# liuyuan-pal/NeRO

Measured on AMD Instinct MI355X. Metric: training rays/sec (Stage-I shape, 128 samples/ray), higher is better.
Workload: dtype f32 (dense layers: fp32 operands carried as exact / block-scaled 16-bit plane pairs or triples on the bf16/fp16 matrix pipe with fp32 accumulation, fp32-grade error; modes {'fwd': 'f16x3', 'tan': 'f16x3', 'bwd': 'f16x3', 'dw': 'f16x3'}); 1 GPU; GlossySynthetic 'bell' Stage-I shape, 4096 rays x (64+64+32) samples per GPU, training-schedule step 25000; rays_per_gpu=4096, parallelism=dp1, optimizer=adam(fused), streams=3, f16_paired_mask=3, fg_table=reference asset (tests/golden/fg_lut_ref.npz)

## Files before the change

nero_amd/csrc/mlp_f16_util.h:

```cpp
#pragma once

#ifdef F16_PHASE_TIMING
__device__ unsigned long long g_phase[16];
#define PH_DECL long long ph_t = clock64(), ph_acc[8] = {0, 0, 0, 0, 0, 0, 0, 0}
#define PH(k) do { __builtin_amdgcn_sched_barrier(0); const long long t_ = clock64(); ph_acc[k] += t_ - ph_t; ph_t = t_; __builtin_amdgcn_sched_barrier(0); } while (0)
#define PH_PARAM , long long& ph_t, long long (&ph_acc)[8]
#define PH_ARG , ph_t, ph_acc
#define PH_END do { if (threadIdx.x == 0) for (int k_ = 0; k_ < 8; ++k_) atomicAdd(&g_phase[k_], (unsigned long long)ph_acc[k_]); } while (0)
#else
#define PH_PARAM
#define PH_ARG
#define PH_DECL
#define PH(k)
#define PH_END
#endif

typedef _Float16 f16x8 __attribute__((ext_vector_type(8)));
typedef _Float16 f16x2 __attribute__((ext_vector_type(2)));
typedef float f32x2 __attribute__((ext_vector_type(2)));
typedef float f32x16 __attribute__((ext_vector_type(16)));

constexpr float BETA = 100.0f;
constexpr int SA = 528;
constexpr int PLANE_A = 64 * SA;
// ... 142 lines not shown
    for (int l = NERO_MAX_LAYERS - 1; l >= 0; --l) {
        const float *pm, *pa;
        images(ch.layer[l], pm, pa);
        if (l < ch.n_layers) { fb = pa ? pa : fb; fb = pm ? pm : fb; }
    }
#pragma unroll
    for (int k = 0; k < WSC_N; ++k) r.v[k] = 1.f;
    if (fb == nullptr) return;
#pragma unroll
    for (int l = 0; l < NERO_MAX_LAYERS; ++l) {
        const float *pm, *pa;
        images(ch.layer[l], pm, pa);
        const bool in = l < ch.n_layers;
        pm = (in && pm) ? pm : fb;
        pa = (in && pa) ? pa : fb;
        r.v[2 * l] = *pm;
        r.v[2 * l + 1] = *pa;
    }
}
__device__ __forceinline__ void wsc_commit(float* wsc, const WscRegs& r, int tid) {
    if (tid == 0) {
#pragma unroll
        for (int k = 0; k < WSC_N; k += 4) *reinterpret_cast<float4*>(wsc + k) = make_float4(r.v[k], r.v[k + 1], r.v[k + 2], r.v[k + 3]);
    }
}

struct WF { uint4 wh, wl; };
struct XF { uint4 xh0, xl0, xh1, xl1; };

__device__ __forceinline__ void load_w(WF& o, const uint4* wp, int c) {
    const uint4* w = wp + (size_t)c * 128;
    o.wh = w[0];
    o.wl = w[64];
}
__device__ __forceinline__ void load_x(XF& o, const char* xp, int half_bytes, int plane_bytes, int c) {
    const char* x = xp + c * 32;
    o.xh0 = *reinterpret_cast<const uint4*>(x);
    o.xl0 = *reinterpret_cast<const uint4*>(x + plane_bytes);
    x += half_bytes;
    o.xh1 = *reinterpret_cast<const uint4*>(x);
    o.xl1 = *reinterpret_cast<const uint4*>(x + plane_bytes);
}
#define NERO_MFH(ACC, A, B) \
    ACC = __builtin_amdgcn_mfma_f32_32x32x16_f16(__builtin_bit_cast(f16x8, A), __builtin_bit_cast(f16x8, B), ACC, 0, 0, 0)
__device__ __forceinline__ void ops_compute(f32x16 (&aH)[2], const WF& w, const XF& x) {
    NERO_MFH(aH[0], w.wl, x.xh0); NERO_MFH(aH[1], w.wl, x.xh1);
    NERO_MFH(aH[0], w.wh, x.xl0); NERO_MFH(aH[1], w.wh, x.xl1);
    NERO_MFH(aH[0], w.wh, x.xh0); NERO_MFH(aH[1], w.wh, x.xh1);
}
#define NERO_FENCE() __builtin_amdgcn_sched_barrier(0)

constexpr int F16_PW_N = 3;
__device__ __forceinline__ void prefetch_w(WF& wa, WF& wb, WF& wc, const uint4* wp, int n, int from = 0) {
    const int last = n - 1;
    if (from <= 0) load_w(wa, wp, 0);
    if (from <= 1) load_w(wb, wp, 1 < last ? 1 : last);
    if (from <= 2) load_w(wc, wp, 2 < last ? 2 : last);
}
__device__ __forceinline__ void gemm_f16x3_loop(f32x16 (&aH)[2], const uint4* wp, const char* xp, int half_bytes,
                                           int plane_bytes, int n, bool pre, WF& wa, WF& wb, WF& wc) {
    if (n <= 0) return;
    WF wd;
    XF xa, xb;
    const int last = n - 1;
#define NERO_CL(c) ((c) < last ? (c) : last)
    prefetch_w(wa, wb, wc, wp, n, pre ? F16_PW_N : 0);
    load_x(xa, xp, half_bytes, plane_bytes, 0);
    NERO_FENCE();
    for (int c = 0; c < n; c += 4) {
        load_w(wd, wp, NERO_CL(c + 3)); load_x(xb, xp, half_bytes, plane_bytes, NERO_CL(c + 1)); NERO_FENCE();
        ops_compute(aH, wa, xa); NERO_FENCE();
        if (c + 1 < n) {
            load_w(wa, wp, NERO_CL(c + 4)); load_x(xa, xp, half_bytes, plane_bytes, NERO_CL(c + 2)); NERO_FENCE();
            ops_compute(aH, wb, xb); NERO_FENCE();
        }
        if (c + 2 < n) {
            load_w(wb, wp, NERO_CL(c + 5)); load_x(xb, xp, half_bytes, plane_bytes, NERO_CL(c + 3)); NERO_FENCE();
            ops_compute(aH, wc, xa); NERO_FENCE();
        }
        if (c + 3 < n) {
            load_w(wc, wp, NERO_CL(c + 6)); load_x(xa, xp, half_bytes, plane_bytes, NERO_CL(c + 4)); NERO_FENCE();
            ops_compute(aH, wd, xb); NERO_FENCE();
        }
    }
#undef NERO_CL
}
__device__ __forceinline__ void gemm_f16x3(f32x16 (&aH)[2], const uint4* wp, const char* xp, int half_bytes, int plane_bytes, int n) {
    WF wa, wb, wc;
    gemm_f16x3_loop(aH, wp, xp, half_bytes, plane_bytes, n, false, wa, wb, wc);
}

struct WF2 { WF a, b; };
__device__ __forceinline__ void load_w2(WF2& o, const uint4* wp0, const uint4* wp1, int c) {
    load_w(o.a, wp0, c);
    load_w(o.b, wp1, c);
}
__device__ __forceinline__ void ops_compute2(f32x16 (&aH0)[2], f32x16 (&aH1)[2], const WF2& w, const XF& x) {
    ops_compute(aH0, w.a, x);
    ops_compute(aH1, w.b, x);
}
__device__ __forceinline__ void gemm_f16x3_dual(f32x16 (&aH0)[2], f32x16 (&aH1)[2], const uint4* wp0,
                                                const uint4* wp1, const char* xp, int half_bytes, int plane_bytes, int n) {
    if (n <= 0) return;
    WF2 w0, w1, w2;
    XF xa, xb;
    const int last = n - 1;
#define NERO_CL(c) ((c) < last ? (c) : last)
#define NERO_K2(W, X) NERO_FENCE(); ops_compute2(aH0, aH1, W, X); NERO_FENCE()
    load_w2(w0, wp0, wp1, 0);
    load_w2(w1, wp0, wp1, NERO_CL(1));
    load_x(xa, xp, half_bytes, plane_bytes, 0);
    NERO_FENCE();
    for (int c = 0; c < n; c += 6) {
        load_w2(w2, wp0, wp1, NERO_CL(c + 2)); load_x(xb, xp, half_bytes, plane_bytes, NERO_CL(c + 1)); NERO_K2(w0, xa);
        if (c + 1 < n) { load_w2(w0, wp0, wp1, NERO_CL(c + 3)); load_x(xa, xp, half_bytes, plane_bytes, NERO_CL(c + 2)); NERO_K2(w1, xb); }
        if (c + 2 < n) { load_w2(w1, wp0, wp1, NERO_CL(c + 4)); load_x(xb, xp, half_bytes, plane_bytes, NERO_CL(c + 3)); NERO_K2(w2, xa); }
        if (c + 3 < n) { load_w2(w2, wp0, wp1, NERO_CL(c + 5)); load_x(xa, xp, half_bytes, plane_bytes, NERO_CL(c + 4)); NERO_K2(w0, xb); }
        if (c + 4 < n) { load_w2(w0, wp0, wp1, NERO_CL(c + 6)); load_x(xb, xp, half_bytes, plane_bytes, NERO_CL(c + 5)); NERO_K2(w1, xa); }
        if (c + 5 < n) { load_w2(w1, wp0, wp1, NERO_CL(c + 7)); load_x(xa, xp, half_bytes, plane_bytes, NERO_CL(c + 6)); NERO_K2(w2, xb); }
    }
#undef NERO_K2
#undef NERO_CL
}

template <int V> struct IC { static constexpr int value = V; };
template <int I, int N, class F> __device__ __forceinline__ void static_for(F&& f) {
    if constexpr (I < N) { f(IC<I>{}); static_for<I + 1, N>(f); }
}
template <int N, class F>
__device__ __forceinline__ void gemm_f16x3_fixed_hook(f32x16 (&aH)[2], const uint4* wp, const char* xp, int half_bytes,
                                                      int plane_bytes, F&& hook) {
    constexpr int XD = 1, XN = XD + 1, WD = 3, WN = WD + 1;
    WF w[WN];
    XF x[XN];
    static_for<0, WD>([&](auto c) { if (c.value < N) load_w(w[c.value], wp, c.value); });
    static_for<0, XD>([&](auto c) { if (c.value < N) load_x(x[c.value], xp, half_bytes, plane_bytes, c.value); });
    NERO_FENCE();
    static_for<0, N>([&](auto cc) {
        constexpr int c = cc.value;
        if (c + WD < N) load_w(w[(c + WD) % WN], wp, c + WD);
        if (c + XD < N) load_x(x[(c + XD) % XN], xp, half_bytes, plane_bytes, c + XD);
        hook(cc);
        NERO_FENCE();
        ops_compute(aH, w[c % WN], x[c % XN]);
        NERO_FENCE();
    });
}
template <int N>
__device__ __forceinline__ void gemm_f16x3_fixed(f32x16 (&aH)[2], const uint4* wp, const char* xp, int half_bytes,
                                                 int plane_bytes) {
    gemm_f16x3_fixed_hook<N>(aH, wp, xp, half_bytes, plane_bytes, [](auto) {});
}

__device__ __forceinline__ void zero2(f32x16 (&acc)[2]) {
#pragma unroll
    for (int r = 0; r < 2; ++r)
#pragma unroll
        for (int v = 0; v < 16; ++v) acc[r][v] = 0.f;
}

template <int ACT>
__device__ __forceinline__ void fwd_values(const f32x16 (&aH)[2], const float4 (&bq)[4], const float (&U)[2], float4 (&val)[2][4],
                                           float (&m)[2]) {
#pragma unroll
    for (int r = 0; r < 2; ++r) {
        m[r] = 0.f;
#pragma unroll
        for (int g = 0; g < 4; ++g) {
            float4 v;
            v.x = act_fwd<ACT>(fmaf(aH[r][4 * g], U[r], bq[g].x));
            v.y = act_fwd<ACT>(fmaf(aH[r][4 * g + 1], U[r], bq[g].y));
            v.z = act_fwd<ACT>(fmaf(aH[r][4 * g + 2], U[r], bq[g].z));
            v.w = act_fwd<ACT>(fmaf(aH[r][4 * g + 3], U[r], bq[g].w));
            val[r][g] = v;
            m[r] = fmaxf(m[r], amax4(v));
        }
    }
}

__device__ __forceinline__ float max_xor32(float m) {
    const auto r = __builtin_amdgcn_permlane32_swap(__float_as_uint(m), __float_as_uint(m), false, false);
    return fmaxf(__uint_as_float(r[0]), __uint_as_float(r[1]));
}
__device__ __forceinline__ unsigned other_half(unsigned v, int h) {
    const auto r = __builtin_amdgcn_permlane32_swap(v, v, false, false);
    return h ? r[0] : r[1];
}
template <int CTRL> __device__ __forceinline__ float dpp_f32(float v) {
    return __uint_as_float(__builtin_amdgcn_update_dpp(0u, __float_as_uint(v), CTRL, 0xf, 0xf, true));
}
__device__ __forceinline__ float max_4lanes(float m) { m = fmaxf(m, dpp_f32<0xB1>(m)); return fmaxf(m, dpp_f32<0x4E>(m)); }
__device__ __forceinline__ float max_8lanes(float m) { m = max_4lanes(m); return fmaxf(m, dpp_f32<0x141>(m)); }
__device__ __forceinline__ float sum_8lanes(float s) { s += dpp_f32<0xB1>(s); s += dpp_f32<0x4E>(s); return s + dpp_f32<0x141>(s); }

__device__ __forceinline__ void publish_rowmax(float* rmax, float m0, float m1, int wave, int i, int h) {
    m0 = max_xor32(m0);
    m1 = max_xor32(m1);
    if (h == 0) { rmax[i * 8 + wave] = m0; rmax[(32 + i) * 8 + wave] = m1; }
}
__device__ __forceinline__ float row_max8(const float* rmax, int row) {
    const float4 a = *reinterpret_cast<const float4*>(rmax + row * 8);
    const float4 b = *reinterpret_cast<const float4*>(rmax + row * 8 + 4);
    return fmaxf(fmaxf(fmaxf(a.x, a.y), fmaxf(a.z, a.w)), fmaxf(fmaxf(b.x, b.y), fmaxf(b.z, b.w)));
}

template <int ACT, bool HEAD, bool PRE>
__device__ __forceinline__ void bwd_values(const float4 (&gq)[2][4], const float4 (&pa)[2][4], size_t goff, bool has_inj,
                                           const nero_bwd_layer& L, int row0, int i, int fbase, int n_rows, float4 (&val)[2][4],
                                           float (&m)[2], const float4 (&ijp)[2][4]) {
    const int nh = L.n_head;
    float4 gs[2][4];
#pragma unroll
    for (int r = 0; r < 2; ++r)
#pragma unroll
        for (int g = 0; g < 4; ++g) gs[r][g] = gq[r][g];
    if (HEAD) {
        float dj[2][4];
#pragma unroll
        for (int r = 0; r < 2; ++r) {
            const float4 dyh = *reinterpret_cast<const float4*>(L.head_dy + (size_t)(row0 + 32 * r + i) * 4);
            dj[r][0] = dyh.x; dj[r][1] = dyh.y; dj[r][2] = dyh.z; dj[r][3] = dyh.w;
        }
#pragma unroll
        for (int g = 0; g < 4; ++g) {
            float4 hw[4];
#pragma unroll
            for (int j = 0; j < 4; ++j) hw[j] = *reinterpret_cast<const float4*>(L.head_w + (j < nh ? j : 0) * NERO_HID + fbase + 8 * g);
#pragma unroll
            for (int r = 0; r < 2; ++r)
#pragma unroll
                for (int j = 0; j < 4; ++j)
                    if (j < nh) {
                        gs[r][g].x = fmaf(dj[r][j], hw[j].x, gs[r][g].x); gs[r][g].y = fmaf(dj[r][j], hw[j].y, gs[r][g].y);
                        gs[r][g].z = fmaf(dj[r][j], hw[j].z, gs[r][g].z); gs[r][g].w = fmaf(dj[r][j], hw[j].w, gs[r][g].w);
                    }
            __builtin_amdgcn_sched_barrier(0);
        }
    }
#pragma unroll
    for (int r = 0; r < 2; ++r) {
        const bool live = (row0 + 32 * r + i) < n_rows;
        float4 ij[4];
        if (PRE) {
#pragma unroll
            for (int g = 0; g < 4; ++g) ij[g] = ijp[r][g];
        } else if (has_inj) {
#pragma unroll
            for (int g = 0; g < 4; ++g) ij[g] = *reinterpret_cast<const float4*>(L.inj + goff + (size_t)r * 32 * NERO_HID + 8 * g);
            if (ACT == NERO_ACT_SOFTPLUS100 && L.inj_adot) {
                float4 ad[4];
#pragma unroll
                for (int g = 0; g < 4; ++g) ad[g] = *reinterpret_cast<const float4*>(L.inj_adot + goff + (size_t)r * 32 * NERO_HID + 8 * g);
#pragma unroll
                for (int g = 0; g < 4; ++g) {
                    const float4 a = pa[r][g];
                    ij[g].x = inj_elem(a.x, ij[g].x, ad[g].x); ij[g].y = inj_elem(a.y, ij[g].y, ad[g].y);
                    ij[g].z = inj_elem(a.z, ij[g].z, ad[g].z); ij[g].w = inj_elem(a.w, ij[g].w, ad[g].w);
                }
            }
        }
        m[r] = 0.f;
#pragma unroll
        for (int g = 0; g < 4; ++g) {
            const float4 a = pa[r][g];
            float4 d;
            d.x = act_grad<ACT>(a.x, gs[r][g].x); d.y = act_grad<ACT>(a.y, gs[r][g].y);
            d.z = act_grad<ACT>(a.z, gs[r][g].z); d.w = act_grad<ACT>(a.w, gs[r][g].w);
            if (has_inj) { d.x += ij[g].x; d.y += ij[g].y; d.z += ij[g].z; d.w += ij[g].w; }
            if (!live) d = make_float4(0.f, 0.f, 0.f, 0.f);
            val[r][g] = d;
            m[r] = fmaxf(m[r], amax4(d));
        }
        __builtin_amdgcn_sched_barrier(0);
    }
}
template <int ACT, bool PRE>
__device__ __forceinline__ void bwd_values_h(const float4 (&gq)[2][4], const float4 (&pa)[2][4], size_t goff, bool has_inj,
                                             const nero_bwd_layer& L, int row0, int i, int fbase, int n_rows, float4 (&val)[2][4],
                                             float (&m)[2], const float4 (&ijp)[2][4]) {
    if (L.n_head > 0) bwd_values<ACT, true, PRE>(gq, pa, goff, has_inj, L, row0, i, fbase, n_rows, val, m, ijp);
    else bwd_values<ACT, false, PRE>(gq, pa, goff, has_inj, L, row0, i, fbase, n_rows, val, m, ijp);
}
```

nero_amd/csrc/mlp_f16p.hip:

```cpp
#include <hip/hip_runtime.h>
#include <stdint.h>
#include "../../include/nero_hip.h"
#include "common.h"
#include "mlp_split.h"

namespace {

#include "mlp_f16_util.h"

constexpr int NW = 4;

struct LdsP { char* actp; float* rs_main; float* rs_aux; float* rmax; float* wsc; char* scr; };
__device__ __forceinline__ LdsP carve_p(char* smem) {
    LdsP l;
    l.actp = smem;
    l.rs_main = reinterpret_cast<float*>(smem + 2 * PLANE_A);
    l.rs_aux = l.rs_main + 64;
    l.rmax = l.rs_aux + 64;
    l.wsc = l.rmax + 64 * 8;
    l.scr = reinterpret_cast<char*>(l.wsc + 32);
    return l;
}
inline int p_lds_bytes() { return 2 * PLANE_A + LDS_SMALL_BYTES + NW * SCRP_BYTES; }

// ... 84 lines not shown
        }
    }
}

__device__ __forceinline__ void gemm_aux_global2(f32x16 (&aH0)[2], f32x16 (&aH1)[2], const uint4* wp0,
                                                 const uint4* wp1, const float* __restrict__ aux, int ld, int k, int n, const Ctx& c, float inv0,
                                                 float inv1) {
    if (n <= 0) return;
    int g0 = c.row0 + c.i, g1 = c.row0 + 32 + c.i;
    g0 = g0 < c.n_rows ? g0 : c.n_rows - 1;
    g1 = g1 < c.n_rows ? g1 : c.n_rows - 1;
    const float* p0 = aux + (size_t)g0 * ld;
    const float* p1 = aux + (size_t)g1 * ld;
    WF2 wa, wb;
    RawX ra, rb;
    XF x;
    load_w2(wa, wp0, wp1, 0);
    load_raw(ra, p0, p1, 0, c.h, k);
    for (int s = 0; s < n; s += 2) {
        if (s + 1 < n) { load_w2(wb, wp0, wp1, s + 1); load_raw(rb, p0, p1, s + 1, c.h, k); }
        NERO_FENCE();
        raw_to_x(x, ra, inv0, inv1);
        ops_compute2(aH0, aH1, wa, x);
        NERO_FENCE();
        if (s + 1 < n) {
            if (s + 2 < n) { load_w2(wa, wp0, wp1, s + 2); load_raw(ra, p0, p1, s + 2, c.h, k); }
            NERO_FENCE();
            raw_to_x(x, rb, inv0, inv1);
            ops_compute2(aH0, aH1, wb, x);
            NERO_FENCE();
        }
    }
}

__device__ __forceinline__ void gemm_tile2(f32x16 (&aH0)[2], f32x16 (&aH1)[2], float (&U)[2], const Ctx& c,
                                           int t, const float* w_main, const float* w_aux, float wsc_main, float wsc_aux, int sm, int sx,
                                           const float* aux, int ld_aux, int k_aux_cols) {
    if (sx > 0) {
        const float wsc = wsc_aux;
        const float ra0 = c.S.rs_aux[c.i], ra1 = c.S.rs_aux[32 + c.i];
        const uint4* wp = reinterpret_cast<const uint4*>(reinterpret_cast<const char*>(w_aux) + HDR_BYTES) + (size_t)t * sx * 128 + c.lane;
        gemm_aux_global2(aH0, aH1, wp, wp + (size_t)NW * sx * 128, aux, ld_aux, k_aux_cols, sx, c, 1.f / ra0, 1.f / ra1);
        U[0] = wsc * ra0;
        U[1] = wsc * ra1;
    }
    if (sm > 0) {
        const float wsc = wsc_main;
        const float u0 = wsc * c.S.rs_main[c.i], u1 = wsc * c.S.rs_main[32 + c.i];
        if (sx > 0) {
            const float r0 = U[0] / u0, r1 = U[1] / u1;
#pragma unroll
            for (int v = 0; v < 16; ++v) {
                aH0[0][v] *= r0; aH0[1][v] *= r1;
                aH1[0][v] *= r0; aH1[1][v] *= r1;
            }
        }
        U[0] = u0;
        U[1] = u1;
        const uint4* wp = reinterpret_cast<const uint4*>(reinterpret_cast<const char*>(w_main) + HDR_BYTES) + (size_t)t * sm * 128 + c.lane;
        gemm_f16x3_dual(aH0, aH1, wp, wp + (size_t)NW * sm * 128, c.S.actp + c.i * SA + 16 * c.h, 32 * SA, PLANE_A, sm);
    }
}

__device__ __forceinline__ void gemm_tile(f32x16 (&aH)[2], float (&U)[2], const Ctx& c, int t, const float* w_main,
                                          const float* w_aux, float wsc_main, float wsc_aux, int sm, int sx, const float* aux, int ld_aux,
                                          int k_aux_cols) {
    if (sx > 0) {
        const float wsc = wsc_aux;
        const float ra0 = c.S.rs_aux[c.i], ra1 = c.S.rs_aux[32 + c.i];
        gemm_aux_global(aH, reinterpret_cast<const uint4*>(reinterpret_cast<const char*>(w_aux) + HDR_BYTES) + (size_t)t * sx * 128 + c.lane,
                        aux, ld_aux, k_aux_cols, sx, c, 1.f / ra0, 1.f / ra1);
        U[0] = wsc * ra0;
        U[1] = wsc * ra1;
    }
    if (sm > 0) {
        const float wsc = wsc_main;
        const float u0 = wsc * c.S.rs_main[c.i], u1 = wsc * c.S.rs_main[32 + c.i];
        if (sx > 0) {
            const float r0 = U[0] / u0, r1 = U[1] / u1;
#pragma unroll
            for (int v = 0; v < 16; ++v) { aH[0][v] *= r0; aH[1][v] *= r1; }
        }
        U[0] = u0;
        U[1] = u1;
        const uint4* wp = reinterpret_cast<const uint4*>(reinterpret_cast<const char*>(w_main) + HDR_BYTES) + (size_t)t * sm * 128 + c.lane;
        gemm_f16x3(aH, wp, c.S.actp + c.i * SA + 16 * c.h, 32 * SA, PLANE_A, sm);
    }
}

__device__ __forceinline__ void eval_head_p(const char* planes, const float* rs, const float* __restrict__ w, const float* __restrict__ b,
                                            float* __restrict__ out, int n_head, int hk, int row0, int tid) {
    const int q = tid & 7;
#pragma unroll
    for (int pass = 0; pass < 8 / NW; ++pass) {
        const int r = (tid >> 3) + 32 * pass;
        float s[4] = {0.f, 0.f, 0.f, 0.f};
        for (int c4 = 4 * q; c4 < hk; c4 += 32) {
            const float4 x = load_planes4h(planes + r * SA + c4 * 2, PLANE_A);
#pragma unroll
            for (int j = 0; j < 4; ++j)
                if (j < n_head) {
                    const float4 ww = *reinterpret_cast<const float4*>(w + j * NERO_HID + c4);
                    s[j] = fmaf(x.x, ww.x, fmaf(x.y, ww.y, fmaf(x.z, ww.z, fmaf(x.w, ww.w, s[j]))));
                }
        }
#pragma unroll
        for (int j = 0; j < 4; ++j) s[j] = sum_8lanes(s[j]);
        if (q == 0) {
            const float sc = rs[r];
#pragma unroll
            for (int j = 0; j < 4; ++j)
                if (j < n_head) out[(size_t)(row0 + r) * 4 + j] = s[j] * sc + (b ? b[j] : 0.f);
        }
    }
}

__device__ __forceinline__ void commit_planes_p(const Ctx& c, const float4 (&v0)[2][4], const float4 (&v1)[2][4], bool live0, bool live1) {
    __syncthreads();
    const int e0 = scale_exp(row_max8(c.S.rmax, c.i)), e1 = scale_exp(row_max8(c.S.rmax, 32 + c.i));
    const float inv0 = pow2i(-e0), inv1 = pow2i(-e1);
    if (live0) {
        char* dst = c.S.actp + c.i * SA + (32 * c.wave + 4 * c.h) * 2;
#pragma unroll
        for (int g = 0; g < 4; ++g) {
            store_planes4h(dst + 16 * g, PLANE_A, scale4(v0[0][g], inv0));
            store_planes4h(dst + 32 * SA + 16 * g, PLANE_A, scale4(v0[1][g], inv1));
        }
    }
    if (live1) {
        char* dst = c.S.actp + c.i * SA + (32 * (c.wave + NW) + 4 * c.h) * 2;
#pragma unroll
        for (int g = 0; g < 4; ++g) {
            store_planes4h(dst + 16 * g, PLANE_A, scale4(v1[0][g], inv0));
            store_planes4h(dst + 32 * SA + 16 * g, PLANE_A, scale4(v1[1][g], inv1));
        }
    }
    if (c.wave == 0 && c.h == 0) { c.S.rs_main[c.i] = pow2i(e0); c.S.rs_main[32 + c.i] = pow2i(e1); }
    __syncthreads();
}

__device__ __forceinline__ Ctx make_ctx(char* smem, int n_rows) {
    Ctx c;
    c.S = carve_p(smem);
    c.lane = threadIdx.x & 63;
    c.wave = __builtin_amdgcn_readfirstlane(threadIdx.x >> 6);
    c.i = c.lane & 31;
    c.h = c.lane >> 5;
    c.row0 = blockIdx.x * 64;
    c.n_rows = n_rows;
    c.scr = reinterpret_cast<float*>(c.S.scr + c.wave * SCRP_BYTES);
    return c;
}

__device__ __forceinline__ void fwd_load_bias(float4 (&bq)[4], const nero_fwd_layer& L, const Ctx& c, int t) {
#pragma unroll
    for (int g = 0; g < 4; ++g)
        bq[g] = L.bias ? *reinterpret_cast<const float4*>(L.bias + 32 * t + 8 * g + 4 * c.h) : make_float4(0.f, 0.f, 0.f, 0.f);
}

__device__ __forceinline__ void fwd_epilogue(const nero_fwd_layer& L, const Ctx& c, int t, const f32x16 (&aH)[2],
                                             const float4 (&bq)[4], const float (&U)[2], float4 (&val)[2][4], float (&m)[2] PH_PARAM) {
    if (L.act == NERO_ACT_RELU) fwd_values<NERO_ACT_RELU>(aH, bq, U, val, m);
    else if (L.act == NERO_ACT_SOFTPLUS100) fwd_values<NERO_ACT_SOFTPLUS100>(aH, bq, U, val, m);
    else fwd_values<NERO_ACT_NONE>(aH, bq, U, val, m);
    PH(3);
    if (L.save) {
        float* sblock = L.save + (size_t)c.row0 * NERO_HID + 32 * t;
        acc_to_global16(c.scr, val[0], sblock, c.lane);
        acc_to_global16(c.scr, val[1], sblock + (size_t)32 * NERO_HID, c.lane);
    }
    if (L.relu_mask) {
#pragma unroll
        for (int r = 0; r < 2; ++r) {
            unsigned bits = 0u;
#pragma unroll
            for (int g = 0; g < 4; ++g) {
                bits |= (val[r][g].x > 0.f ? 1u : 0u) << (4 * g);
                bits |= (val[r][g].y > 0.f ? 1u : 0u) << (4 * g + 1);
                bits |= (val[r][g].z > 0.f ? 1u : 0u) << (4 * g + 2);
                bits |= (val[r][g].w > 0.f ? 1u : 0u) << (4 * g + 3);
            }
            const unsigned other = other_half(bits, c.h);
            if (c.h == 0) L.relu_mask[(size_t)(c.row0 + 32 * r + c.i) * 8 + t] = bits | (other << 16);
        }
    }
    publish_rowmax(c.S.rmax, m[0], m[1], t, c.i, c.h);
    PH(4);
}

__device__ __forceinline__ void fwd_tile(const nero_fwd_chain& ch, const nero_fwd_layer& L, int l, const Ctx& c, int t, float4 (&val)[2][4],
                                         float (&m)[2] PH_PARAM) {
    m[0] = m[1] = 0.f;
    if (t < L.n_tiles) {
        f32x16 aH[2];
        zero2(aH);
        float4 bq[4];
        fwd_load_bias(bq, L, c, t);
        float U[2] = {1.f, 1.f};
        PH(1);
        gemm_tile(aH, U, c, t, L.w_main, L.w_aux, c.S.wsc[2 * l], c.S.wsc[2 * l + 1], L.k_main >> 4, L.k_aux >> 4, ch.aux, ch.ld_aux, ch.k_aux);
        PH(2);
        fwd_epilogue(L, c, t, aH, bq, U, val, m PH_ARG);
    } else {
        publish_rowmax(c.S.rmax, 0.f, 0.f, t, c.i, c.h);
        PH(4);
    }
}

__device__ __forceinline__ void fwd_tile_pair(const nero_fwd_chain& ch, const nero_fwd_layer& L, int l, const Ctx& c, int t, float4 (&v0)[2][4],
                                              float4 (&v1)[2][4], float (&m0)[2], float (&m1)[2] PH_PARAM) {
    f32x16 aH0[2], aH1[2];
    zero2(aH0);
    zero2(aH1);
    float4 bq[4];
    fwd_load_bias(bq, L, c, t);
    float U[2] = {1.f, 1.f};
    PH(1);
    gemm_tile2(aH0, aH1, U, c, t, L.w_main, L.w_aux, c.S.wsc[2 * l], c.S.wsc[2 * l + 1], L.k_main >> 4, L.k_aux >> 4, ch.aux,
                   ch.ld_aux, ch.k_aux);
    float4 bq1[4];
    fwd_load_bias(bq1, L, c, t + NW);
    PH(2);
    fwd_epilogue(L, c, t, aH0, bq, U, v0, m0 PH_ARG);
    fwd_epilogue(L, c, t + NW, aH1, bq1, U, v1, m1 PH_ARG);
}

__global__ __launch_bounds__(NW * 64, 2) void fwd_p_kernel(nero_fwd_chain ch, int n_rows) {
    extern __shared__ __attribute__((aligned(16))) char smem[];
    const Ctx c = make_ctx(smem, n_rows);
    const int tid = threadIdx.x;
    PH_DECL;
#ifdef F16_PHASE_TIMING
    const long long ph_start = ph_t;
#endif
    WscRegs wr;
    wsc_request(wr, ch, [](const nero_fwd_layer& Lx, const float*& pm, const float*& pa) { pm = Lx.k_main > 0 && Lx.n_tiles > 0 ? Lx.w_main : nullptr; pa = Lx.k_aux > 0 && Lx.n_tiles > 0 ? Lx.w_aux : nullptr; });
    if (ch.init) load_planes_scaled_p(c.S.actp, c.S.rs_main, ch.init, ch.ld_init, ch.k_init, c.row0, n_rows, tid);
    if (ch.aux) aux_row_scales_p(c.S.rs_aux, ch.aux, ch.ld_aux, ch.k_aux, c.row0, n_rows, tid);
    wsc_commit(c.S.wsc, wr, tid);
    __syncthreads();
    PH(0);
    for (int l = 0; l < ch.n_layers; ++l) {
        const nero_fwd_layer L = load_layer(ch, l);
        if (L.n_head > 0) eval_head_p(c.S.actp, c.S.rs_main, L.head_w, L.head_b, L.head_out, L.n_head, L.head_k, c.row0, tid);
        if (L.n_tiles == 0) continue;
        float4 v0[2][4], v1[2][4];
        float m0[2], m1[2];
        if (c.wave + NW < L.n_tiles) fwd_tile_pair(ch, L, l, c, c.wave, v0, v1, m0, m1 PH_ARG);
        else {
            fwd_tile(ch, L, l, c, c.wave, v0, m0 PH_ARG);
            fwd_tile(ch, L, l, c, c.wave + NW, v1, m1 PH_ARG);
        }
        commit_planes_p(c, v0, v1, c.wave < L.n_tiles, c.wave + NW < L.n_tiles);
        PH(5);
    }
#ifdef F16_PHASE_TIMING
    ph_acc[7] = clock64() - ph_start;
    ph_acc[6] = 0;
#endif
    PH_END;
}

__device__ __forceinline__ void tan_epilogue(const nero_tan_layer& L, const Ctx& c, int t, const f32x16 (&aH)[2],
                                             const float (&U)[2], float4 (&val)[2][4], float (&m)[2]) {
    const size_t goff = (size_t)(c.row0 + c.i) * NERO_HID + 32 * t + 4 * c.h;
    const size_t boff = (size_t)c.row0 * NERO_HID + 32 * t;
    const bool want_inj = L.inj != nullptr;
    m[0] = m[1] = 0.f;
    NERO_FENCE();
    float4 pa[2][4], pg[2][4];
#pragma unroll
    for (int r = 0; r < 2; ++r)
#pragma unroll
        for (int g = 0; g < 4; ++g) {
            pa[r][g] = *reinterpret_cast<const float4*>(L.a_saved + goff + (size_t)r * 32 * NERO_HID + 8 * g);
            pg[r][g] = make_float4(0.f, 0.f, 0.f, 0.f);
        }
    if (want_inj) {
#pragma unroll
        for (int r = 0; r < 2; ++r)
#pragma unroll
            for (int g = 0; g < 4; ++g) pg[r][g] = *reinterpret_cast<const float4*>(L.gbar + goff + (size_t)r * 32 * NERO_HID + 8 * g);
    }
    float* scr = c.scr;
#pragma unroll
    for (int r = 0; r < 2; ++r) {
        const bool live = (c.row0 + 32 * r + c.i) < c.n_rows;
        float4 ijq[4], adq[4];
#pragma unroll
        for (int g = 0; g < 4; ++g) {
            const float4 a = pa[r][g], gb = pg[r][g];
            float4 ad, ij;
            tan_elem(a.x, aH[r][4 * g] * U[r], gb.x, live, ad.x, ij.x);
            tan_elem(a.y, aH[r][4 * g + 1] * U[r], gb.y, live, ad.y, ij.y);
            tan_elem(a.z, aH[r][4 * g + 2] * U[r], gb.z, live, ad.z, ij.z);
            tan_elem(a.w, aH[r][4 * g + 3] * U[r], gb.w, live, ad.w, ij.w);
            val[r][g] = ad;
            m[r] = fmaxf(m[r], amax4(ad));
            adq[g] = live ? ad : make_float4(0.f, 0.f, 0.f, 0.f);
            ijq[g] = ij;
        }
        acc_to_global16(scr, adq, L.adot + boff + (size_t)r * 32 * NERO_HID, c.lane);
        if (want_inj) acc_to_global16(scr, ijq, L.inj + boff + (size_t)r * 32 * NERO_HID, c.lane);
    }
    publish_rowmax(c.S.rmax, m[0], m[1], t, c.i, c.h);
}

__device__ __forceinline__ void tan_tile(const nero_tan_chain& ch, const nero_tan_layer& L, int l, const Ctx& c, int t, float4 (&val)[2][4],
                                         float (&m)[2]) {
    if (t < L.n_tiles) {
        f32x16 aH[2];
        zero2(aH);
        float U[2] = {1.f, 1.f};
        gemm_tile(aH, U, c, t, L.w_main, L.w_aux, c.S.wsc[2 * l], c.S.wsc[2 * l + 1], L.k_main >> 4, L.k_aux >> 4, ch.aux, ch.ld_aux, ch.k_aux);
        tan_epilogue(L, c, t, aH, U, val, m);
    } else {
        m[0] = m[1] = 0.f;
        publish_rowmax(c.S.rmax, 0.f, 0.f, t, c.i, c.h);
    }
}

__device__ __forceinline__ void tan_tile_pair(const nero_tan_chain& ch, const nero_tan_layer& L, int l, const Ctx& c, int t, float4 (&v0)[2][4],
                                              float4 (&v1)[2][4], float (&m0)[2], float (&m1)[2]) {
    f32x16 aH0[2], aH1[2];
    zero2(aH0);
    zero2(aH1);
    float U[2] = {1.f, 1.f};
    gemm_tile2(aH0, aH1, U, c, t, L.w_main, L.w_aux, c.S.wsc[2 * l], c.S.wsc[2 * l + 1], L.k_main >> 4, L.k_aux >> 4, ch.aux,
                   ch.ld_aux, ch.k_aux);
    tan_epilogue(L, c, t, aH0, U, v0, m0);
    tan_epilogue(L, c, t + NW, aH1, U, v1, m1);
}

__global__ __launch_bounds__(NW * 64, 2) void tan_p_kernel(nero_tan_chain ch, int n_rows) {
    extern __shared__ __attribute__((aligned(16))) char smem[];
    const Ctx c = make_ctx(smem, n_rows);
    const int tid = threadIdx.x;
    WscRegs wr;
    wsc_request(wr, ch, [](const nero_tan_layer& Lx, const float*& pm, const float*& pa) { pm = Lx.k_main > 0 ? Lx.w_main : nullptr; pa = Lx.k_aux > 0 ? Lx.w_aux : nullptr; });
    if (ch.init) load_planes_scaled_p(c.S.actp, c.S.rs_main, ch.init, ch.ld_init, ch.k_init, c.row0, n_rows, tid);
    if (ch.aux) aux_row_scales_p(c.S.rs_aux, ch.aux, ch.ld_aux, ch.k_aux, c.row0, n_rows, tid);
    wsc_commit(c.S.wsc, wr, tid);
    __syncthreads();
    for (int l = 0; l < ch.n_layers; ++l) {
        const nero_tan_layer L = load_layer(ch, l);
        float4 v0[2][4], v1[2][4];
        float m0[2], m1[2];
        if (c.wave + NW < L.n_tiles) tan_tile_pair(ch, L, l, c, c.wave, v0, v1, m0, m1);
        else {
            tan_tile(ch, L, l, c, c.wave, v0, m0);
            tan_tile(ch, L, l, c, c.wave + NW, v1, m1);
        }
        commit_planes_p(c, v0, v1, c.wave < L.n_tiles, c.wave + NW < L.n_tiles);
    }
}

__device__ __forceinline__ void combine_acc(float4 (&gq)[2][4], const f32x16 (&aH)[2], const float (&u)[2]) {
#pragma unroll
    for (int r = 0; r < 2; ++r)
#pragma unroll
        for (int g = 0; g < 4; ++g)
            gq[r][g] = make_float4(aH[r][4 * g] * u[r], aH[r][4 * g + 1] * u[r],
                                   aH[r][4 * g + 2] * u[r], aH[r][4 * g + 3] * u[r]);
}

template <bool MASKS>
__device__ __forceinline__ void bwd_tile(const nero_bwd_chain& ch, const nero_bwd_layer& L, int l, const Ctx& c, int t, bool first, float rs0, float rs1,
                                         float4 (&val)[2][4], float (&m)[2]) {
    m[0] = m[1] = 0.f;
    const bool live_t = t < L.k_main_tiles;
    const int fbase = 32 * t + 4 * c.h;
    const size_t goff = (size_t)(c.row0 + c.i) * NERO_HID + fbase;
    const size_t boff = (size_t)c.row0 * NERO_HID + 32 * t;
    const int steps = L.n_out >> 4;
    const bool has_inj = !MASKS && !first && L.inj != nullptr;
    const char* xp = c.S.actp + c.i * SA + 16 * c.h;
    float4 pa[2][4];
    auto load_pa = [&]() {
        if (first || !live_t) return;
        if (MASKS && L.act_prev != NERO_ACT_RELU) return;
        if (MASKS || (L.mask_prev && L.act_prev == NERO_ACT_RELU)) {
#pragma unroll
            for (int r = 0; r < 2; ++r) {
                const unsigned bits = L.mask_prev[(size_t)(c.row0 + 32 * r + c.i) * 8 + t] >> (16 * c.h);
#pragma unroll
                for (int g = 0; g < 4; ++g)
                    pa[r][g] = make_float4((bits >> (4 * g)) & 1u ? 1.f : 0.f, (bits >> (4 * g + 1)) & 1u ? 1.f : 0.f,
                                           (bits >> (4 * g + 2)) & 1u ? 1.f : 0.f, (bits >> (4 * g + 3)) & 1u ? 1.f : 0.f);
            }
        } else if (!MASKS) {
#pragma unroll
            for (int r = 0; r < 2; ++r)
#pragma unroll
                for (int g = 0; g < 4; ++g) pa[r][g] = *reinterpret_cast<const float4*>(L.a_prev + goff + (size_t)r * 32 * NERO_HID + 8 * g);
        }
    };
    float4 gq[2][4];
    if (L.n_out > 0) {
        f32x16 aH[2];
        if (ch.d_aux && L.w_aux_t && t < L.k_aux_tiles) {
            zero2(aH);
            const float wsc = c.S.wsc[2 * l + 1];
            gemm_f16x3(aH, reinterpret_cast<const uint4*>(reinterpret_cast<const char*>(L.w_aux_t) + HDR_BYTES) + (size_t)t * steps * 128 + c.lane,
                       xp, 32 * SA, PLANE_A, steps);
            const float u[2] = {wsc * rs0, wsc * rs1};
            combine_acc(gq, aH, u);
            int li = c.i, lf = fbase;
            P_LOCAL_V(li);
            P_LOCAL_V(lf);
#pragma unroll
            for (int r = 0; r < 2; ++r)
#pragma unroll
                for (int g = 0; g < 4; ++g) {
                    const int f = lf + 8 * g;
                    if (f < ch.ld_daux) *reinterpret_cast<float4*>(ch.d_aux + (size_t)(c.row0 + 32 * r + li) * ch.ld_daux + f) = gq[r][g];
                }
        }
        if (!live_t || (first && !ch.d_init)) { publish_rowmax(c.S.rmax, 0.f, 0.f, t, c.i, c.h); return; }
        load_pa();
        NERO_FENCE();
        zero2(aH);
        const float wsc = c.S.wsc[2 * l];
        gemm_f16x3(aH, reinterpret_cast<const uint4*>(reinterpret_cast<const char*>(L.w_main_t) + HDR_BYTES) + (size_t)t * steps * 128 + c.lane,
                   xp, 32 * SA, PLANE_A, steps);
        const float u[2] = {wsc * rs0, wsc * rs1};
        combine_acc(gq, aH, u);
        if (first) {
            if (ch.d_init) {
                const int ldi = ch.ld_dinit;
                int li = c.i, lf = fbase;
                P_LOCAL_V(li);
                P_LOCAL_V(lf);
#pragma unroll
                for (int r = 0; r < 2; ++r)
#pragma unroll
                    for (int g = 0; g < 4; ++g) {
                        const int f = lf + 8 * g;
                        if (f < ldi) {
                            float4 v = gq[r][g];
                            float4* dstp = reinterpret_cast<float4*>(ch.d_init + (size_t)(c.row0 + 32 * r + li) * ldi + f);
                            if (ch.accumulate_dinit) { const float4 o = *dstp; v.x += o.x; v.y += o.y; v.z += o.z; v.w += o.w; }
                            *dstp = v;
                        }
                    }
            }
            return;
        }
    } else {
        if (!live_t) { publish_rowmax(c.S.rmax, 0.f, 0.f, t, c.i, c.h); return; }
        load_pa();
#pragma unroll
        for (int g = 0; g < 4; ++g) {
            gq[0][g] = scale4(load_planes4h(c.S.actp + c.i * SA + (fbase + 8 * g) * 2, PLANE_A), rs0);
            gq[1][g] = scale4(load_planes4h(c.S.actp + (32 + c.i) * SA + (fbase + 8 * g) * 2, PLANE_A), rs1);
        }
    }
    float4 ijp[2][4];
#pragma unroll
    for (int r = 0; r < 2; ++r)
#pragma unroll
        for (int g = 0; g < 4; ++g) ijp[r][g] = make_float4(0.f, 0.f, 0.f, 0.f);
    if (L.act_prev == NERO_ACT_RELU) bwd_values_h<NERO_ACT_RELU, false>(gq, pa, goff, has_inj, L, c.row0, c.i, fbase, c.n_rows, val, m, ijp);
    else if (!MASKS && L.act_prev == NERO_ACT_SOFTPLUS100) bwd_values_h<NERO_ACT_SOFTPLUS100, false>(gq, pa, goff, has_inj, L, c.row0, c.i, fbase, c.n_rows, val, m, ijp);
    else bwd_values_h<NERO_ACT_NONE, false>(gq, pa, goff, has_inj, L, c.row0, c.i, fbase, c.n_rows, val, m, ijp);
    if (L.delta_prev) {
        acc_to_global16(c.scr, val[0], L.delta_prev + boff, c.lane);
        acc_to_global16(c.scr, val[1], L.delta_prev + boff + (size_t)32 * NERO_HID, c.lane);
    }
    publish_rowmax(c.S.rmax, m[0], m[1], t, c.i, c.h);
}

template <bool MASKS>
__global__ __launch_bounds__(NW * 64, 2) void bwd_p_kernel(nero_bwd_chain ch, int n_rows) {
    extern __shared__ __attribute__((aligned(16))) char smem[];
    const Ctx c = make_ctx(smem, n_rows);
    const int tid = threadIdx.x;
    WscRegs wr;
    wsc_request(wr, ch, [](const nero_bwd_layer& Lx, const float*& pm, const float*& pa) { pm = Lx.n_out > 0 ? Lx.w_main_t : nullptr; pa = Lx.n_out > 0 ? Lx.w_aux_t : nullptr; });
    if (ch.dy) load_planes_scaled_p(c.S.actp, c.S.rs_main, ch.dy, ch.ld_dy, ch.k_dy, c.row0, n_rows, tid);
    else {
        for (int idx = tid; idx < 2 * PLANE_A / 16; idx += NW * 64) reinterpret_cast<uint4*>(c.S.actp)[idx] = make_uint4(0u, 0u, 0u, 0u);
        if (tid < 64) c.S.rs_main[tid] = 1.f;
    }
    wsc_commit(c.S.wsc, wr, tid);
    __syncthreads();
    for (int l = ch.n_layers - 1; l >= 0; --l) {
        const nero_bwd_layer L = load_layer(ch, l);
        const bool first = (L.a_prev == nullptr);
        if (first && ch.d_init == nullptr && !(ch.d_aux && L.w_aux_t)) break;
        if (first && L.n_out == 0) break;
        const float rs0 = c.S.rs_main[c.i], rs1 = c.S.rs_main[32 + c.i];
        float4 v0[2][4], v1[2][4];
        float m0[2], m1[2];
        bwd_tile<MASKS>(ch, L, l, c, c.wave, first, rs0, rs1, v0, m0);
        bwd_tile<MASKS>(ch, L, l, c, c.wave + NW, first, rs0, rs1, v1, m1);
        if (first) break;
        commit_planes_p(c, v0, v1, c.wave < L.k_main_tiles, c.wave + NW < L.k_main_tiles);
    }
}

}

#ifdef F16_PHASE_TIMING
extern "C" int nero_debug_phases_p(unsigned long long* out16, int reset) {
    hipDeviceSynchronize();
    if (out16) hipMemcpyFromSymbol(out16, HIP_SYMBOL(g_phase), sizeof(unsigned long long) * 16);
    if (reset) { unsigned long long z[16] = {0}; hipMemcpyToSymbol(HIP_SYMBOL(g_phase), z, sizeof(z)); }
    return 0;
}
#endif
template <auto K, class CH> static void launch_p(const CH* ch, int n_rows, hipStream_t stream) {
    NERO_ONCE(hipFuncSetAttribute((const void*)K, hipFuncAttributeMaxDynamicSharedMemorySize, p_lds_bytes()));
    nero_prof_mark_paired();
    hipLaunchKernelGGL(K, dim3((n_rows + 63) / 64), dim3(NW * 64), p_lds_bytes(), stream, *ch, n_rows);
}
int nero_f16p_forward(const nero_fwd_chain* ch, int n_rows, hipStream_t stream) {
    for (int l = 0; l < ch->n_layers; ++l)
        if ((ch->layer[l].k_main | ch->layer[l].k_aux) & 15)
            return nero_fail(NERO_ERR_ARG, "nero_mlp_forward(f16x3p): k_main / k_aux must be multiples of 16");
    launch_p<fwd_p_kernel>(ch, n_rows, stream);
    return NERO_OK;
}

int nero_f16p_tangent(const nero_tan_chain* ch, int n_rows, hipStream_t stream) {
    for (int l = 0; l < ch->n_layers; ++l)
        if ((ch->layer[l].k_main | ch->layer[l].k_aux) & 15)
            return nero_fail(NERO_ERR_ARG, "nero_mlp_tangent(f16x3p): k_main / k_aux must be multiples of 16");
    launch_p<tan_p_kernel>(ch, n_rows, stream);
    return NERO_OK;
}

bool nero_f16p_masks_only(const nero_bwd_chain* ch) {
    for (int l = 0; l < ch->n_layers; ++l) {
        const nero_bwd_layer& L = ch->layer[l];
        if (L.inj || L.inj_adot) return false;
        if (L.a_prev == nullptr) continue;
        if (L.act_prev == NERO_ACT_NONE) continue;
        if (!(L.act_prev == NERO_ACT_RELU && L.mask_prev)) return false;
    }
    return true;
}
int nero_f16p_backward(const nero_bwd_chain* ch, int n_rows, hipStream_t stream) {
    for (int l = 0; l < ch->n_layers; ++l)
        if (ch->layer[l].n_out & 15) return nero_fail(NERO_ERR_ARG, "nero_mlp_backward(f16x3p): n_out must be a multiple of 16");
    if (ch->d_aux && (ch->ld_daux & 3)) return nero_fail(NERO_ERR_ARG, "nero_mlp_backward(f16x3p): ld_daux must be a multiple of 4");
    if (ch->d_init && (ch->ld_dinit & 3)) return nero_fail(NERO_ERR_ARG, "nero_mlp_backward(f16x3p): ld_dinit must be a multiple of 4");
    if (nero_f16p_masks_only(ch)) launch_p<bwd_p_kernel<true>>(ch, n_rows, stream);
    else launch_p<bwd_p_kernel<false>>(ch, n_rows, stream);
    return NERO_OK;
}
```

Measured before the change: 154,900 rays/s.

## Pipeline weight loads across plain MLP layers with inline-asm prefetch rings

Adds a fast path in the forward MLP kernel for plain hidden layers: weights for the next layer are prefetched into registers before the current layer's outputs are stored, and a three-slot ring of inline-asm global loads with explicit vmcnt waits feeds the dual-tile f16x3 GEMM. The backward masked path uses a similar fixed-length four-deep weight ring. The goal is to hide global weight-load latency between layers and to replace compiler-scheduled waits with precise counters. In exchange it adds hand-counted waitcnt logic (including outstanding store counts) that is fragile if store counts or layouts change, and it raises register pressure.

```diff
diff --git a/nero_amd/csrc/mlp_f16_util.h b/nero_amd/csrc/mlp_f16_util.h
--- a/nero_amd/csrc/mlp_f16_util.h
+++ b/nero_amd/csrc/mlp_f16_util.h
@@ -318,6 +318,97 @@
     gemm_f16x3_fixed_hook<N>(aH, wp, xp, half_bytes, plane_bytes, [](auto) {});
 }
 
+typedef unsigned u32x4 __attribute__((ext_vector_type(4)));
+struct WQ2 { u32x4 ah, al, bh, bl; };
+constexpr int WQ_STEP_BYTES = 2048, WQ_PLANE_BYTES = 1024;
+template <int C, bool ORDER_MEM>
+__device__ __forceinline__ void load_w2q(WQ2& o, unsigned voff, const char* s0, const char* s1) {
+    const char* p0 = s0 + C * WQ_STEP_BYTES;
+    const char* p1 = s1 + C * WQ_STEP_BYTES;
+#define NERO_W2Q_ASM "s_nop 4\n\tglobal_load_dwordx4 %0, %4, %5\n\tglobal_load_dwordx4 %1, %4, %5 offset:1024\n\t" \
+                     "global_load_dwordx4 %2, %4, %6\n\tglobal_load_dwordx4 %3, %4, %6 offset:1024"
+    if (ORDER_MEM) asm volatile(NERO_W2Q_ASM : "=&v"(o.ah), "=&v"(o.al), "=&v"(o.bh), "=&v"(o.bl) : "v"(voff), "s"(p0), "s"(p1) : "memory");
+    else asm volatile(NERO_W2Q_ASM : "=&v"(o.ah), "=&v"(o.al), "=&v"(o.bh), "=&v"(o.bl) : "v"(voff), "s"(p0), "s"(p1));
+#undef NERO_W2Q_ASM
+}
+static_assert(WQ_PLANE_BYTES == 1024, "offset:1024 in load_w2q");
+template <int N> __device__ __forceinline__ void wait_vm() { asm volatile("s_waitcnt vmcnt(%0)" : : "n"(N)); }
+__device__ __forceinline__ void landed_w2q(WQ2& w) {
+    NERO_FENCE();
+    asm volatile("" : "+v"(w.ah), "+v"(w.al), "+v"(w.bh), "+v"(w.bl));
+}
+__device__ __forceinline__ void ops_compute2q(f32x16 (&aH0)[2], f32x16 (&aH1)[2], const WQ2& w, const XF& x) {
+    NERO_MFH(aH0[0], w.al, x.xh0); NERO_MFH(aH0[1], w.al, x.xh1);
+    NERO_MFH(aH0[0], w.ah, x.xl0); NERO_MFH(aH0[1], w.ah, x.xl1);
+    NERO_MFH(aH0[0], w.ah, x.xh0); NERO_MFH(aH0[1], w.ah, x.xh1);
+    NERO_MFH(aH1[0], w.bl, x.xh0); NERO_MFH(aH1[1], w.bl, x.xh1);
+    NERO_MFH(aH1[0], w.bh, x.xl0); NERO_MFH(aH1[1], w.bh, x.xl1);
+    NERO_MFH(aH1[0], w.bh, x.xh0); NERO_MFH(aH1[1], w.bh, x.xh1);
+}
+__device__ __forceinline__ void prefill_w2q(WQ2& r0, WQ2& r1, unsigned voff, const char* s0, const char* s1) {
+    load_w2q<0, true>(r0, voff, s0, s1);
+    load_w2q<1, true>(r1, voff, s0, s1);
+    NERO_FENCE();
+}
+constexpr int PRE_STORES = 2 * 2 * (32 / SCRP_ROWS) * (SCRP_ROWS / 8);
+template <int N>
+__device__ __forceinline__ void gemm_f16x3_dual_fixed(f32x16 (&aH0)[2], f32x16 (&aH1)[2], unsigned voff, const char* s0, const char* s1,
+                                                      const char* xp, int half_bytes, int plane_bytes, WQ2& r0, WQ2& r1, bool stores_behind) {
+    static_assert(N >= 3, "ring of three");
+    WQ2 r2;
+    XF x[2];
+    load_x(x[0], xp, half_bytes, plane_bytes, 0);
+    NERO_FENCE();
+    static_for<0, N>([&](auto cc) {
+        constexpr int c = cc.value;
+        auto slot = [&](auto k) -> WQ2& { if constexpr (k.value % 3 == 0) return r0; else if constexpr (k.value % 3 == 1) return r1; else return r2; };
+        if constexpr (c + 2 < N) load_w2q<c + 2, false>(slot(IC<c + 2>{}), voff, s0, s1);
+        if constexpr (c + 1 < N) load_x(x[(c + 1) & 1], xp, half_bytes, plane_bytes, c + 1);
+        NERO_FENCE();
+        constexpr int later = 4 * ((c + 1 < N ? 1 : 0) + (c + 2 < N ? 1 : 0));
+        if (c < 2 && stores_behind) wait_vm<later + PRE_STORES>();
+        else wait_vm<later>();
+        landed_w2q(slot(cc));
+        ops_compute2q(aH0, aH1, slot(cc), x[c & 1]);
+        NERO_FENCE();
+    });
+}
+
+struct WQ1 { u32x4 h, l; };
+template <int C> __device__ __forceinline__ void load_w1q(WQ1& o, unsigned voff, const char* s) {
+    const char* p = s + C * WQ_STEP_BYTES;
+    asm volatile("s_nop 4\n\tglobal_load_dwordx4 %0, %2, %3\n\tglobal_load_dwordx4 %1, %2, %3 offset:1024"
+                 : "=&v"(o.h), "=&v"(o.l) : "v"(voff), "s"(p));
+}
+__device__ __forceinline__ void landed_w1q(WQ1& w) {
+    NERO_FENCE();
+    asm volatile("" : "+v"(w.h), "+v"(w.l));
+}
+template <int N>
+__device__ __forceinline__ void gemm_f16x3_single_fixed(f32x16 (&aH)[2], unsigned voff, const char* s, const char* xp, int half_bytes,
+                                                        int plane_bytes) {
+    constexpr int WD = 3, WN = WD + 1;
+    static_assert(N > WD, "ring of four");
+    WQ1 w[WN];
+    XF x[2];
+    static_for<0, WD>([&](auto cc) { load_w1q<cc.value>(w[cc.value], voff, s); });
+    load_x(x[0], xp, half_bytes, plane_bytes, 0);
+    NERO_FENCE();
+    static_for<0, N>([&](auto cc) {
+        constexpr int c = cc.value;
+        if constexpr (c + WD < N) load_w1q<c + WD>(w[(c + WD) % WN], voff, s);
+        if constexpr (c + 1 < N) load_x(x[(c + 1) & 1], xp, half_bytes, plane_bytes, c + 1);
+        NERO_FENCE();
+        constexpr int later = 2 * ((c + 1 < N ? 1 : 0) + (c + 2 < N ? 1 : 0) + (c + 3 < N ? 1 : 0));
+        wait_vm<later>();
+        landed_w1q(w[c % WN]);
+        NERO_MFH(aH[0], w[c % WN].l, x[c & 1].xh0); NERO_MFH(aH[1], w[c % WN].l, x[c & 1].xh1);
+        NERO_MFH(aH[0], w[c % WN].h, x[c & 1].xl0); NERO_MFH(aH[1], w[c % WN].h, x[c & 1].xl1);
+        NERO_MFH(aH[0], w[c % WN].h, x[c & 1].xh0); NERO_MFH(aH[1], w[c % WN].h, x[c & 1].xh1);
+        NERO_FENCE();
+    });
+}
+
 __device__ __forceinline__ void zero2(f32x16 (&acc)[2]) {
 #pragma unroll
     for (int r = 0; r < 2; ++r)
diff --git a/nero_amd/csrc/mlp_f16p.hip b/nero_amd/csrc/mlp_f16p.hip
--- a/nero_amd/csrc/mlp_f16p.hip
+++ b/nero_amd/csrc/mlp_f16p.hip
@@ -260,18 +260,29 @@
     return c;
 }
 
+__device__ __forceinline__ Ctx relane(const Ctx& c) {
+    Ctx r = c;
+    int lane = c.lane;
+    P_LOCAL_V(lane);
+    r.lane = lane;
+    r.i = lane & 31;
+    r.h = lane >> 5;
+    return r;
+}
+
 __device__ __forceinline__ void fwd_load_bias(float4 (&bq)[4], const nero_fwd_layer& L, const Ctx& c, int t) {
 #pragma unroll
     for (int g = 0; g < 4; ++g)
         bq[g] = L.bias ? *reinterpret_cast<const float4*>(L.bias + 32 * t + 8 * g + 4 * c.h) : make_float4(0.f, 0.f, 0.f, 0.f);
 }
 
-__device__ __forceinline__ void fwd_epilogue(const nero_fwd_layer& L, const Ctx& c, int t, const f32x16 (&aH)[2],
-                                             const float4 (&bq)[4], const float (&U)[2], float4 (&val)[2][4], float (&m)[2] PH_PARAM) {
-    if (L.act == NERO_ACT_RELU) fwd_values<NERO_ACT_RELU>(aH, bq, U, val, m);
-    else if (L.act == NERO_ACT_SOFTPLUS100) fwd_values<NERO_ACT_SOFTPLUS100>(aH, bq, U, val, m);
+__device__ __forceinline__ void fwd_act_values(int act, const f32x16 (&aH)[2], const float4 (&bq)[4], const float (&U)[2], float4 (&val)[2][4],
+                                               float (&m)[2]) {
+    if (act == NERO_ACT_RELU) fwd_values<NERO_ACT_RELU>(aH, bq, U, val, m);
+    else if (act == NERO_ACT_SOFTPLUS100) fwd_values<NERO_ACT_SOFTPLUS100>(aH, bq, U, val, m);
     else fwd_values<NERO_ACT_NONE>(aH, bq, U, val, m);
-    PH(3);
+}
+__device__ __forceinline__ void fwd_outputs(const nero_fwd_layer& L, const Ctx& c, int t, const float4 (&val)[2][4], const float (&m)[2]) {
     if (L.save) {
         float* sblock = L.save + (size_t)c.row0 * NERO_HID + 32 * t;
         acc_to_global16(c.scr, val[0], sblock, c.lane);
@@ -293,6 +304,12 @@
         }
     }
     publish_rowmax(c.S.rmax, m[0], m[1], t, c.i, c.h);
+}
+__device__ __forceinline__ void fwd_epilogue(const nero_fwd_layer& L, const Ctx& c, int t, const f32x16 (&aH)[2],
+                                             const float4 (&bq)[4], const float (&U)[2], float4 (&val)[2][4], float (&m)[2] PH_PARAM) {
+    fwd_act_values(L.act, aH, bq, U, val, m);
+    PH(3);
+    fwd_outputs(L, c, t, val, m);
     PH(4);
 }
 
@@ -310,6 +327,10 @@
         PH(2);
         fwd_epilogue(L, c, t, aH, bq, U, val, m PH_ARG);
     } else {
+#pragma unroll
+        for (int r = 0; r < 2; ++r)
+#pragma unroll
+            for (int g = 0; g < 4; ++g) val[r][g] = make_float4(0.f, 0.f, 0.f, 0.f);
         publish_rowmax(c.S.rmax, 0.f, 0.f, t, c.i, c.h);
         PH(4);
     }
@@ -333,9 +354,65 @@
     fwd_epilogue(L, c, t + NW, aH1, bq1, U, v1, m1 PH_ARG);
 }
 
+__device__ __forceinline__ bool fwd_plain_layer(const nero_fwd_chain& ch, int l, int wave) {
+    return l < ch.n_layers && ch.layer[l].k_main == NERO_HID && ch.layer[l].k_aux == 0 && ch.layer[l].n_head == 0 &&
+           wave + NW < ch.layer[l].n_tiles;
+}
+__device__ __forceinline__ const char* w16_tile(const float* w, int t) {
+    return reinterpret_cast<const char*>(w) + HDR_BYTES + (size_t)t * (NERO_HID / 16) * WQ_STEP_BYTES;
+}
+__device__ __forceinline__ int fwd_plain_run(const nero_fwd_chain& ch, int l, const Ctx& c0 PH_PARAM) {
+    const Ctx c = relane(c0);
+    const int t = c.wave;
+    const unsigned voff = 16u * c.lane;
+    WQ2 r0, r1;
+    {
+        const float* w = ch.layer[l].w_main;
+        PIN_P(w);
+        prefill_w2q(r0, r1, voff, w16_tile(w, t), w16_tile(w, t + NW));
+    }
+    bool stores_behind = false;
+    for (;;) {
+        const nero_fwd_layer L = load_layer(ch, l);
+        const Ctx c = relane(c0);
+        f32x16 aH0[2], aH1[2];
+        zero2(aH0);
+        zero2(aH1);
+        float4 bq[4];
+        fwd_load_bias(bq, L, c, t);
+        const float wsc = c.S.wsc[2 * l];
+        const float U[2] = {wsc * c.S.rs_main[c.i], wsc * c.S.rs_main[32 + c.i]};
+        PH(1);
+        gemm_f16x3_dual_fixed<NERO_HID / 16>(aH0, aH1, voff, w16_tile(L.w_main, t), w16_tile(L.w_main, t + NW),
+                                             c.S.actp + c.i * SA + 16 * c.h, 32 * SA, PLANE_A, r0, r1, stores_behind);
+        float4 bq1[4];
+        fwd_load_bias(bq1, L, c, t + NW);
+        PH(2);
+        float4 v0[2][4], v1[2][4];
+        float m0[2], m1[2];
+        fwd_act_values(L.act, aH0, bq, U, v0, m0);
+        fwd_act_values(L.act, aH1, bq1, U, v1, m1);
+        PH(3);
+        const bool more = fwd_plain_layer(ch, l + 1, c.wave);
+        if (more) {
+            const float* w = ch.layer[l + 1].w_main;
+            PIN_P(w);
+            prefill_w2q(r0, r1, voff, w16_tile(w, t), w16_tile(w, t + NW));
+        }
+        stores_behind = L.save != nullptr;
+        fwd_outputs(L, c, t, v0, m0);
+        fwd_outputs(L, c, t + NW, v1, m1);
+        PH(4);
+        commit_planes_p(c, v0, v1, true, true);
+        PH(5);
+        ++l;
+        if (!more) return l;
+    }
+}
+
 __global__ __launch_bounds__(NW * 64, 2) void fwd_p_kernel(nero_fwd_chain ch, int n_rows) {
     extern __shared__ __attribute__((aligned(16))) char smem[];
-    const Ctx c = make_ctx(smem, n_rows);
+    const Ctx c0 = make_ctx(smem, n_rows), c = c0;
     const int tid = threadIdx.x;
     PH_DECL;
 #ifdef F16_PHASE_TIMING
@@ -348,16 +425,23 @@
     wsc_commit(c.S.wsc, wr, tid);
     __syncthreads();
     PH(0);
-    for (int l = 0; l < ch.n_layers; ++l) {
+    for (int l = 0; l < ch.n_layers;) {
+        if (fwd_plain_layer(ch, l, c0.wave)) {
+            l = fwd_plain_run(ch, l, c0 PH_ARG);
+            PIN_S(l);
+            continue;
+        }
         const nero_fwd_layer L = load_layer(ch, l);
+        const Ctx c = relane(c0);
+        ++l;
         if (L.n_head > 0) eval_head_p(c.S.actp, c.S.rs_main, L.head_w, L.head_b, L.head_out, L.n_head, L.head_k, c.row0, tid);
         if (L.n_tiles == 0) continue;
         float4 v0[2][4], v1[2][4];
         float m0[2], m1[2];
-        if (c.wave + NW < L.n_tiles) fwd_tile_pair(ch, L, l, c, c.wave, v0, v1, m0, m1 PH_ARG);
+        if (c.wave + NW < L.n_tiles) fwd_tile_pair(ch, L, l - 1, c, c.wave, v0, v1, m0, m1 PH_ARG);
         else {
-            fwd_tile(ch, L, l, c, c.wave, v0, m0 PH_ARG);
-            fwd_tile(ch, L, l, c, c.wave + NW, v1, m1 PH_ARG);
+            fwd_tile(ch, L, l - 1, c, c.wave, v0, m0 PH_ARG);
+            fwd_tile(ch, L, l - 1, c, c.wave + NW, v1, m1 PH_ARG);
         }
         commit_planes_p(c, v0, v1, c.wave < L.n_tiles, c.wave + NW < L.n_tiles);
         PH(5);
@@ -473,6 +557,13 @@
 }
 
 template <bool MASKS>
+__device__ __forceinline__ void bwd_gemm(f32x16 (&aH)[2], const float* w_t, int t, int steps, const char* xp, int lane) {
+    if (MASKS && steps == NERO_HID / 16) gemm_f16x3_single_fixed<NERO_HID / 16>(aH, 16u * lane, w16_tile(w_t, t), xp, 32 * SA, PLANE_A);
+    else gemm_f16x3(aH, reinterpret_cast<const uint4*>(reinterpret_cast<const char*>(w_t) + HDR_BYTES) + (size_t)t * steps * 128 + lane, xp,
+                    32 * SA, PLANE_A, steps);
+}
+
+template <bool MASKS>
 __device__ __forceinline__ void bwd_tile(const nero_bwd_chain& ch, const nero_bwd_layer& L, int l, const Ctx& c, int t, bool first, float rs0, float rs1,
                                          float4 (&val)[2][4], float (&m)[2]) {
     m[0] = m[1] = 0.f;
@@ -509,8 +600,7 @@
         if (ch.d_aux && L.w_aux_t && t < L.k_aux_tiles) {
             zero2(aH);
             const float wsc = c.S.wsc[2 * l + 1];
-            gemm_f16x3(aH, reinterpret_cast<const uint4*>(reinterpret_cast<const char*>(L.w_aux_t) + HDR_BYTES) + (size_t)t * steps * 128 + c.lane,
-                       xp, 32 * SA, PLANE_A, steps);
+            bwd_gemm<MASKS>(aH, L.w_aux_t, t, steps, xp, c.lane);
             const float u[2] = {wsc * rs0, wsc * rs1};
             combine_acc(gq, aH, u);
             int li = c.i, lf = fbase;
@@ -529,8 +619,7 @@
         NERO_FENCE();
         zero2(aH);
         const float wsc = c.S.wsc[2 * l];
-        gemm_f16x3(aH, reinterpret_cast<const uint4*>(reinterpret_cast<const char*>(L.w_main_t) + HDR_BYTES) + (size_t)t * steps * 128 + c.lane,
-                   xp, 32 * SA, PLANE_A, steps);
+        bwd_gemm<MASKS>(aH, L.w_main_t, t, steps, xp, c.lane);
         const float u[2] = {wsc * rs0, wsc * rs1};
         combine_acc(gq, aH, u);
         if (first) {
```

Result: faster. 157,500 rays/s, median of 6 (+1.7%).
